# revdotcom/paper_accurate_fast_cheap

Hardware: AMD Instinct MI355X
Metric: audio-sec/sec (1/RTF) GigaSpeech long-form encode (higher is better)
Workload: dtype f32+bf16-slot

## Files before the change

### include/pafc_encoder_ops.h

```cpp
#ifndef PAFC_ENCODER_OPS_H
#define PAFC_ENCODER_OPS_H

#include "pafc_wkv6.h"

#ifdef __cplusplus
extern "C" {
#endif

int pafc_dwconv1d_cl(int dtype, int B, int T_in, int C, int K, int left_pad, int T_out, const void *x,
                     const void *w, const void *bias, void *y, int glu, const int32_t *lens,
                     pafc_stream_t stream);

int pafc_dwconv1d_cl_ex(int dtype, int B, int T_in, int C, int K, int left_pad, int T_out, const void *x, long ldx,
                        const void *w, const void *bias, void *y, int act, const int32_t *lens, pafc_stream_t stream);

int pafc_dwconv1d_cl_ln_silu(int dtype, int B, int T_in, int C, int K, int left_pad, int T_out, const void *x, long ldx,
                             const void *w, const void *bias, const void *gamma, const void *beta, float eps, void *y,
                             const int32_t *lens, pafc_stream_t stream);

size_t pafc_dwconv1d_cl_wgrad_workspace_bytes(int B, int T_out, int C, int K);
int pafc_dwconv1d_cl_wgrad(int dtype, int B, int T_in, int C, int K, int left_pad, int T_out, const void *x, long ldx,
                           const void *dy, float *dw, float *dbias, void *workspace, size_t workspace_bytes,
                           pafc_stream_t stream);

// ... 149 lines not shown
int pafc_mamba2_scan_skip_bf16(int B, int L, int H, const void *xbc, long ldx, const float *dt, const float *log_a,
                               const float *D, void *y_bf16, int reverse, int chunk_len, void *workspace,
                               size_t workspace_bytes, pafc_stream_t stream);
int pafc_mamba2_gate_norm(int dtype, long rows, int d_inner, const void *y, const void *z, long ld_z,
                          const void *norm_weight, float eps, void *out, pafc_stream_t stream);

int pafc_gemm_bf16(long M, int N, int K, int batch, const void *A, long lda, long strideA, const void *W, long ldw,
                   long strideW, const void *bias, long strideBias, const void *residual, long ldr, long strideR,
                   void *out, long ldo, long strideO, float alpha, int act, pafc_stream_t stream);
int pafc_gemm_bf16_glu_half(long M, int N, int K, int batch);
int pafc_conv3x3s2_nhwc_bf16_ph(int B, int T1, int F1, int Ci, int Co, const void *in, const void *w_tap_co_ci, const void *bias,
                                void *out, int relu, int tile_m, pafc_stream_t stream);
int pafc_gemm_bf16_ph(long M, int N, int K, int batch, const void *A, long lda, long strideA, const void *W, long ldw,
                      long strideW, const void *bias, long strideBias, const void *residual, long ldr, long strideR,
                      void *out, long ldo, long strideO, float alpha, int act, int tile_n, int tile_m, pafc_stream_t stream);
int pafc_gemm_ph_ex(long M, int N, int K, int batch, const void *A, long lda, long strideA, int a_split, const void *W, long ldw,
                    long strideW, const void *bias, long strideBias, const void *residual, int res_kind, long ldr, long strideR,
                    void *out, int out_kind, long ldo, long lo_off, long strideO, float alpha, int act, int tile_m,
                    pafc_stream_t stream);
int pafc_gemm_ph_ex2(long M, int N, int K, int batch, const void *A, long lda, long strideA, int a_split, int a_plane_block,
                     const void *W, long ldw, long strideW, const void *bias, long strideBias, const void *residual, int res_kind,
                     long ldr, long strideR, void *out, int out_kind, long ldo, long lo_off, long strideO, float alpha, int act,
                     int tile_m, pafc_stream_t stream);
int pafc_conv3x3s2_nhwc_split_ph(int B, int T1, int F1, int Ci, int Co, const void *in_planes, const void *w3_tap_co_3ci,
                                 const float *bias, void *out_planes, int relu, int tile_m, pafc_stream_t stream);

int pafc_residual_dropout(int backward, int dtype_x, int dtype_y, long n, const void *x, const void *y, void *out, float scale,
                          float p, unsigned long long seed, unsigned long long offset, pafc_stream_t stream);
int pafc_silu_dropout(int backward, int dtype, long n, const void *h, const void *dout, void *out, float p,
                      unsigned long long seed, unsigned long long offset, pafc_stream_t stream);

int pafc_multi_transpose_bf16(const void *table, int n, int total_tiles, pafc_stream_t stream);
int pafc_multi_cast_bf16(const void *table, int n, int total_chunks, pafc_stream_t stream);

#ifdef __cplusplus
}
#endif
#endif
```

### paper_accurate_fast_cheap_amd/csrc/gemm_bf16.hip

```cpp
#include <stdio.h>
#include <stdlib.h>

#include "pafc_common.h"
#include "../../include/pafc_encoder_ops.h"

namespace pafc {
namespace {

constexpr int GBM = 128, GBN = 128, GBK = 64;
typedef float f32x4g __attribute__((ext_vector_type(4)));
typedef __bf16 bf16x8g __attribute__((ext_vector_type(8)));

struct GemmParams {
    const bf16_t *A, *W, *bias, *res;
    bf16_t *out;
    long M;
    int N, K;
    long lda, ldw, ldo, ldr;
    long sA, sW, sO, sB, sR;
    float alpha;
    int act;
    int mtiles, ntiles;
    int nk1, K1;
    int pb_sh;
// ... 285 lines not shown
                        (bf16_t)f32_to_bf16_bits(apply_act(fmaf(acc[i][j][g], p.alpha, bv), p.act));
        }
        __syncthreads();
        constexpr int CPR = BN / 8, RPP = 256 / CPR;
#pragma unroll
        for (int q = 0; q < BM / RPP; ++q) {
            const int row = q * RPP + tid / CPR, c8 = (tid % CPR) * 8;
            const long m = m0 + row;
            if (m < p.M && n0 + c8 < p.N)
                *reinterpret_cast<uint4 *>(Oz + m * p.ldo + n0 + c8) = *reinterpret_cast<const uint4 *>(O + row * LDO + c8);
        }
    }
}

}
}

extern "C" int pafc_gemm_bf16_ph(long M, int N, int K, int batch, const void *A, long lda, long strideA, const void *W, long ldw,
                                 long strideW, const void *bias, long strideBias, const void *residual, long ldr, long strideR,
                                 void *out, long ldo, long strideO, float alpha, int act, int tile_n, int tile_m,
                                 pafc_stream_t stream);

static int ph_tile_m(long M, int N, int K, int batch, int act, bool has_residual) {
    if (N % 8 || K % 128 || N < 256) return 0;
    if (act == 4 && N % 256) return 0;
    if (has_residual && act != 0) return 0;
    const int cus = pafc::device_cus();
    const long nt = (N + 255) / 256;
    static const long min_fill = [] { const char *e = getenv("PAFC_PH_MIN_FILL"); return e ? atol(e) : 0L; }();
    if (min_fill > 0) {
        if (((M + 255) / 256) * nt * batch * 100 < (long)cus * min_fill) return 0;
    } else if (((M + 127) / 128) * ((N + 127) / 128) * batch <= 2L * cus) {
        return 0;
    }
    long best_cost = -1;
    int best = 0;
    for (int tm = 256; tm >= 192; tm -= 64) {
        const long tiles = ((M + tm - 1) / tm) * nt * batch;
        const long cost = ((tiles + cus - 1) / cus) * (tm + 64);
        if (best_cost < 0 || cost < best_cost) { best_cost = cost; best = tm; }
    }
    return best;
}

extern "C" int pafc_gemm_bf16_glu_half(long M, int N, int K, int batch) { return ph_tile_m(M, N, K, batch, 4, false) ? 32 : 64; }

extern "C" int pafc_gemm_bf16(long M, int N, int K, int batch, const void *A, long lda, long strideA, const void *W,
                              long ldw, long strideW, const void *bias, long strideBias, const void *residual, long ldr,
                              long strideR, void *out, long ldo, long strideO, float alpha, int act,
                              pafc_stream_t stream) {
    if (!A || !W || !out) return PAFC_ERR_NULL_POINTER;
    if (M <= 0 || N <= 0 || K <= 0 || batch <= 0 || batch > 65535) return PAFC_ERR_BAD_DIMS;
    if (N % 8 || K % pafc::GBK) return PAFC_ERR_UNSUPPORTED;
    if (act < 0 || act > 4) return PAFC_ERR_UNSUPPORTED;
    if (const int tm = ph_tile_m(M, N, K, batch, act, residual != nullptr)) {
        const int rc = pafc_gemm_bf16_ph(M, N, K, batch, A, lda, strideA, W, ldw, strideW, bias, strideBias, residual, ldr, strideR,
                                         out, ldo, strideO, alpha, act, 256, tm, stream);
        if (rc != PAFC_ERR_UNSUPPORTED) return rc;
        if (act == 4) return PAFC_ERR_UNSUPPORTED;
    }
    const bool glu = act == 4;
    if (glu && (N % pafc::GBN || residual)) return PAFC_ERR_UNSUPPORTED;
    if (lda < K || ldw < K || ldo < (glu ? N / 2 : N) || (residual && ldr < N)) return PAFC_ERR_BAD_DIMS;
    if ((lda | ldw | ldo | strideA | strideW | strideO) % 8 || (residual && ((ldr | strideR) % 8))) return PAFC_ERR_ALIGNMENT;
    if ((((uintptr_t)A | (uintptr_t)W | (uintptr_t)out | (uintptr_t)residual) & 15) != 0) return PAFC_ERR_ALIGNMENT;
    pafc::GemmParams p{};
    p.A = (const pafc::bf16_t *)A; p.W = (const pafc::bf16_t *)W; p.bias = (const pafc::bf16_t *)bias;
    p.res = (const pafc::bf16_t *)residual; p.out = (pafc::bf16_t *)out;
    p.M = M; p.N = N; p.K = K;
    p.lda = lda; p.ldw = ldw; p.ldo = ldo; p.ldr = ldr;
    p.sA = strideA; p.sW = strideW; p.sO = strideO; p.sB = strideBias; p.sR = strideR;
    p.alpha = alpha; p.act = act;
    const long cus = pafc::device_cus();
    auto tiles = [&](int bm, int bn) { return ((M + bm - 1) / bm) * ((N + bn - 1) / bn) * (long)batch; };
    int bm = 128, bn = 128;
    if (!glu && tiles(128, 128) * 5 < 7 * cus) {
        if (tiles(128, 64) >= 2 * cus) bn = 64;
        else { bm = 64; bn = 64; }
// ... 187 lines not shown
```

### paper_accurate_fast_cheap_amd/csrc/gemm_ph.hip

```cpp
#include <climits>
#include <cstdlib>
#include <cstring>
#include <type_traits>

#include "pafc_common.h"
#include "../../include/pafc_encoder_ops.h"

namespace pafc {
namespace {

typedef float f32x4p __attribute__((ext_vector_type(4)));
typedef __bf16 bf16x8p __attribute__((ext_vector_type(8)));
typedef unsigned u32x4p __attribute__((ext_vector_type(4)));

struct PhParams {
    const bf16_t *A, *W;
    const void *bias;
    const void *res;
    void *out;
    long M;
    int N, K;
    long lda, ldw, ldo, ldr;
    long sA, sW, sO, sB, sR;
    float alpha;
    int mtiles, ntiles;
    int tm;
    int batch;
    int nk1, pb_shift;
    long pb_bytes;
    int nsteps, a_lo, w_lo;
    int w_step;
    long lo_off;
    float *ln_stats;
    const float *ln_csum;
    float ln_eps, ln_inv_c;
    int T1, F1, T2, F2, Ci, CiA, CiW, spt, inv_spt;
    long in_bytes;
#ifdef PH_STAMPS
    unsigned long long *stamps;
#endif
};

#ifdef PH_STAMPS
#define PH_STAMP(i) do { if (stamp_on) st[(i)] = __builtin_amdgcn_s_memtime(); } while (0)
#else
#define PH_STAMP(i) do { } while (0)
#endif

__device__ __forceinline__ void dma16(__amdgpu_buffer_rsrc_t rsrc, unsigned lane_off, unsigned uniform_off, void *lds_wave_base) {
    __builtin_amdgcn_raw_ptr_buffer_load_lds(rsrc, (__attribute__((address_space(3))) void *)lds_wave_base, 16, lane_off,
// ... 34 lines not shown
__global__ __launch_bounds__(512, 2) void gemm_ph_kernel(const PhParams p) {
    constexpr int BN = PBN;
    constexpr int UA = 128 * 128;
    constexpr int UB = (BN / 2) * 128;
    constexpr int STEP = 2 * UA + 2 * UB;
    constexpr int OFF_A0 = 0, OFF_A1 = UA, OFF_B0 = 2 * UA, OFF_B1 = 2 * UA + UB;
    constexpr int TN = 2;
    constexpr int DA = UA / 8192;
    constexpr int DB = UB / 8192;
    constexpr int OSZ = OUT == 1 ? 4 : 2;
    constexpr bool BIASF32 = OUT != 0;
    constexpr int NST = 8 * (GLU ? 1 : 2) * (OUT == 0 ? 1 : 2) + (LNF == 2 ? 8 : 0);
    static_assert(LNF == 0 || (OUT == 0 && !CONV), "LayerNorm folding: bf16 GEMMs");
    static_assert(!SPL || LNF == 0, "shared-fragment split operands: not with a folded LayerNorm");
    static_assert(LNF != 1 || (RES == 0 && (GLU || ACT == 1)), "LNF 1: the w_1 (SiLU) / pointwise_conv1 (GLU) projections");
    static_assert(LNF != 2 || RES == 1, "LNF 2: a residual GEMM");
    static_assert(!(GLU && (ACT != 0 || RES != 0)), "GLU excludes an activation and a residual");
    static_assert(!(RES != 0 && ACT != 0), "the layer never pairs a residual with an activation");
    extern __shared__ __attribute__((aligned(1024))) unsigned char lds[];

    const int tid = threadIdx.x, lane = tid & 63;
    const int wave = __builtin_amdgcn_readfirstlane(tid >> 6);
    const int wr = wave >> 2, wc = wave & 3;
    const long nblk = (long)p.mtiles * p.ntiles;
    const long total = nblk * p.batch;
    const long per = total / 8;
    const int nt = SPL ? p.nsteps : p.K / PBK;

    auto pix_off = [&](long m) -> long {
        const long tf = (long)p.T2 * p.F2;
        const long bb = m / tf, rem = m - bb * tf;
        const long t2 = rem / p.F2, f2 = rem - t2 * p.F2;
        return (((bb * p.T1 + 2 * t2) * p.F1 + 2 * f2) * p.CiA) * 2;
    };

    struct Tile {
        long m0;
        int n0, z, vr;
        __amdgpu_buffer_rsrc_t Ar, Wr;
    };
    auto make_tile = [&](long t, Tile &T) {
        const bool real = t < total;
        long tt = real ? t : 0;
        if (tt < per * 8) tt = (tt % 8) * per + tt / 8;
        T.z = (int)(tt / nblk);
        const long bid = tt % nblk;
        const int mt0 = (int)(bid / p.ntiles), nt0 = (int)(bid % p.ntiles);
        T.m0 = (long)mt0 * p.tm;
        T.n0 = nt0 * BN;
        T.vr = (int)min((long)p.tm, p.M - T.m0);
        if constexpr (CONV) {
            const long a_base = pix_off(T.m0);
            T.Ar = make_rsrc(reinterpret_cast<const unsigned char *>(p.A) + a_base, real ? p.in_bytes - a_base : 0);
            T.Wr = make_rsrc(p.W + (long)T.n0 * p.CiW, real ? ((long)8 * p.N + p.N - T.n0) * p.CiW * 2 : 0);
        } else {
            T.Ar = make_rsrc(p.A + T.z * p.sA + T.m0 * p.lda, real ? (p.M - T.m0) * p.lda * 2 : 0);
            T.Wr = make_rsrc(p.W + T.z * p.sW + (long)T.n0 * p.ldw, real ? ((long)(p.N - 1 - T.n0) * p.ldw + p.K) * 2 : 0);
        }
    };

    unsigned a_off[2][DA], b_off[2][DB];
    auto a_offsets = [&](const Tile &T, int h) {
        int sl = lane;
        asm volatile("" : "+v"(sl));
        const int sub = sl >> 3, pch = sl & 7;
#pragma unroll
        for (int j = 0; j < DA; ++j) {
            const int u = (wave * DA + j) * 8 + sub;
            const int row = (u >> 6) * 128 + h * 64 + (u & 63);
            const int sc = pch ^ sub;
            const unsigned coff = SPL ? (unsigned)(16 * (sc & 3) + (sc >> 2) * p.a_lo) : (unsigned)(16 * sc);
            a_off[h][j] = CONV ? (unsigned)(pix_off(T.m0 + row) - pix_off(T.m0)) + coff
                               : (unsigned)((long)row * p.lda * 2) + coff;
        }
    };
    auto b_offsets = [&]() {
        const int sub = lane >> 3, pch = lane & 7;
#pragma unroll
        for (int h = 0; h < 2; ++h)
// ... 446 lines not shown
    first = false;
    if constexpr (CONV) make_tile(t + gridDim.x, cur);
    else cur = nxt;
    PH_STAMP(53);
    }
    PH_WAIT(0);
}

template <bool GLU, int ACT, int RES, int OUT, bool CONV = false, int LNF = 0, bool SPL = false>
int launch_ph(const PhParams &p, int batch, hipStream_t s) {
    constexpr size_t lds = 2 * (2 * 128 * 128 + 2 * (PBN / 2) * 128) + 8 * 1024 + (LNF == 1 ? 8 * 1024 + 16 * 1024 : 0);
    auto kern = gemm_ph_kernel<GLU, ACT, RES, OUT, CONV, LNF, SPL>;
    static bool attr_set[64];
    int dev = 0;
    if (hipGetDevice(&dev) != hipSuccess) return PAFC_ERR_LAUNCH;
    if (dev < 0 || dev >= 64 || !attr_set[dev]) {
        if (hipFuncSetAttribute((const void *)kern, hipFuncAttributeMaxDynamicSharedMemorySize, (int)lds) != hipSuccess)
            return PAFC_ERR_LAUNCH;
        if (dev >= 0 && dev < 64) attr_set[dev] = true;
    }
    const int cus = device_cus();
    PhParams q = p;
    q.batch = batch;
    const long total = (long)p.mtiles * p.ntiles * batch;
    const long grid = total < cus ? total : cus;
    hipLaunchKernelGGL(kern, dim3((unsigned)grid), dim3(512), lds, s, q);
    return hipGetLastError() == hipSuccess ? PAFC_OK : PAFC_ERR_LAUNCH;
}

int g_split_walk = -1;
bool split_shared_fragments() {
    if (g_split_walk < 0) {
        const char *e = getenv("PAFC_SPLIT_WALK");
        g_split_walk = !(e && std::strcmp(e, "hilohi") == 0);
    }
    return g_split_walk != 0;
}

}
}

extern "C" int pafc_gemm_ph_ex(long M, int N, int K, int batch, const void *A, long lda, long strideA, int a_split, const void *W,
                               long ldw, long strideW, const void *bias, long strideBias, const void *residual, int res_kind,
                               long ldr, long strideR, void *out, int out_kind, long ldo, long lo_off, long strideO, float alpha,
                               int act, int tile_m, pafc_stream_t stream) {
    return pafc_gemm_ph_ex2(M, N, K, batch, A, lda, strideA, a_split, 0, W, ldw, strideW, bias, strideBias, residual, res_kind, ldr,
                            strideR, out, out_kind, ldo, lo_off, strideO, alpha, act, tile_m, stream);
}

extern "C" int pafc_gemm_ph_ex2(long M, int N, int K, int batch, const void *A, long lda, long strideA, int a_split,
                                int a_plane_block, const void *W, long ldw, long strideW, const void *bias, long strideBias,
                                const void *residual, int res_kind, long ldr, long strideR, void *out, int out_kind, long ldo,
                                long lo_off, long strideO, float alpha, int act, int tile_m, pafc_stream_t stream) {
    if (!A || !W || !out) return PAFC_ERR_NULL_POINTER;
    if (M <= 0 || N <= 0 || K <= 0 || batch <= 0 || batch > 65535) return PAFC_ERR_BAD_DIMS;
    if (act < 0 || act > 4 || out_kind < 0 || out_kind > 2 || res_kind < 0 || res_kind > 2) return PAFC_ERR_UNSUPPORTED;
    if (!residual) res_kind = 0;
    else if (res_kind == 0) return PAFC_ERR_BAD_DIMS;
    const bool glu = act == 4;
    if (tile_m < 64 || tile_m > 256 || tile_m % 64) return PAFC_ERR_UNSUPPORTED;
    if (N % 8 || K % 128) return PAFC_ERR_UNSUPPORTED;
    if (glu && (N % 256 || residual)) return PAFC_ERR_UNSUPPORTED;
    if (residual && act != 0) return PAFC_ERR_UNSUPPORTED;
    if (res_kind == 1 && out_kind != 0) return PAFC_ERR_UNSUPPORTED;
    if (res_kind == 2 && out_kind != 1) return PAFC_ERR_UNSUPPORTED;
    const int Kw = a_split ? 3 * K : K;
    const int No = glu ? N / 2 : N;
    if (lda < (a_split ? 2 * K : K) || ldw < Kw || (residual && ldr < N)) return PAFC_ERR_BAD_DIMS;
    if (out_kind == 2 ? (lo_off < No || ldo < lo_off + No) : ldo < No) return PAFC_ERR_BAD_DIMS;
    if ((lda | ldw | strideA | strideW) % 8 || (ldo | strideO | lo_off) % 8 || (residual && ((ldr | strideR) % 8))) return PAFC_ERR_ALIGNMENT;
    if ((((uintptr_t)A | (uintptr_t)W | (uintptr_t)out | (uintptr_t)residual | (uintptr_t)bias) & 15) != 0) return PAFC_ERR_ALIGNMENT;
    if ((double)M * lda * 2 >= 2.0e9 || (double)N * ldw * 2 >= 2.0e9) return PAFC_ERR_UNSUPPORTED;
    if ((double)256 * ldo * 4 >= 2.0e9 || (residual && (double)256 * ldr * 4 >= 2.0e9)) return PAFC_ERR_UNSUPPORTED;
    pafc::PhParams p{};
    p.A = (const pafc::bf16_t *)A; p.W = (const pafc::bf16_t *)W; p.bias = bias; p.res = residual; p.out = out;
    p.M = M; p.N = N; p.K = Kw;
    p.lda = lda; p.ldw = ldw; p.ldo = ldo; p.ldr = ldr;
    p.sA = strideA; p.sW = strideW; p.sO = strideO; p.sB = strideBias; p.sR = strideR;
    p.alpha = alpha;
    p.nk1 = a_split ? K / 64 : INT_MAX / 4;
    p.pb_shift = 31;
    p.pb_bytes = (long)K * 2;
    if (a_split && a_plane_block) {
        int sh = 0;
        while ((64 << sh) < a_plane_block) ++sh;
        if ((64 << sh) != a_plane_block || K % a_plane_block) return PAFC_ERR_UNSUPPORTED;
        p.pb_shift = sh;
        p.pb_bytes = (long)a_plane_block * 2;
    }
    p.lo_off = lo_off;
    p.tm = tile_m;
    p.mtiles = (int)((M + tile_m - 1) / tile_m);
    p.ntiles = (N + 255) / 256;
    if ((long)p.mtiles * p.ntiles > 0x7fffffffL) return PAFC_ERR_BAD_DIMS;
    hipStream_t s = (hipStream_t)stream;
    if (a_split && out_kind != 0 && pafc::split_shared_fragments() && (double)2 * K * 2 + 64 < 2.0e9) {
        p.nsteps = K / 32;
        p.a_lo = (int)p.pb_bytes;
        p.w_lo = 2 * K * 2;
        p.w_step = 64;
        p.pb_shift = p.pb_shift >= 30 ? 30 : p.pb_shift + 1;
        if (out_kind == 1) {
            if (glu) return pafc::launch_ph<true, 0, 0, 1, false, 0, true>(p, batch, s);
            if (res_kind == 2) return pafc::launch_ph<false, 0, 2, 1, false, 0, true>(p, batch, s);
            if (act == 0) return pafc::launch_ph<false, 0, 0, 1, false, 0, true>(p, batch, s);
            return PAFC_ERR_UNSUPPORTED;
        }
        if (glu || residual) return PAFC_ERR_UNSUPPORTED;
        if (act == 1) return pafc::launch_ph<false, 1, 0, 2, false, 0, true>(p, batch, s);
        if (act == 0) return pafc::launch_ph<false, 0, 0, 2, false, 0, true>(p, batch, s);
        return PAFC_ERR_UNSUPPORTED;
    }
    if (out_kind == 0) {
        if (glu) return pafc::launch_ph<true, 0, 0, 0>(p, batch, s);
        if (res_kind == 1) return pafc::launch_ph<false, 0, 1, 0>(p, batch, s);
        switch (act) {
            case 1: return pafc::launch_ph<false, 1, 0, 0>(p, batch, s);
            case 2: return pafc::launch_ph<false, 2, 0, 0>(p, batch, s);
            case 3: return pafc::launch_ph<false, 3, 0, 0>(p, batch, s);
            default: return pafc::launch_ph<false, 0, 0, 0>(p, batch, s);
        }
    }
    if (out_kind == 1) {
        if (glu) return pafc::launch_ph<true, 0, 0, 1>(p, batch, s);
        if (res_kind == 2) return pafc::launch_ph<false, 0, 2, 1>(p, batch, s);
        if (act == 0) return pafc::launch_ph<false, 0, 0, 1>(p, batch, s);
        return PAFC_ERR_UNSUPPORTED;
    }
    if (glu || residual) return PAFC_ERR_UNSUPPORTED;
    if (act == 1) return pafc::launch_ph<false, 1, 0, 2>(p, batch, s);
    if (act == 0) return pafc::launch_ph<false, 0, 0, 2>(p, batch, s);
    return PAFC_ERR_UNSUPPORTED;
}

extern "C" int pafc_gemm_bf16_ph_ln(long M, int N, int K, const void *A, long lda, const void *W, long ldw, const void *bias,
                                    const void *residual, long ldr, void *out, long ldo, float alpha, int act, int ln_mode,
                                    float *stats, const float *csum, int ln_c, float ln_eps, int tile_m, pafc_stream_t stream) {
    if (!A || !W || !out || !stats) return PAFC_ERR_NULL_POINTER;
    if (M <= 0 || N <= 0 || K <= 0 || ln_c <= 0) return PAFC_ERR_BAD_DIMS;
    if (tile_m < 64 || tile_m > 256 || tile_m % 64) return PAFC_ERR_UNSUPPORTED;
    if (N % 8 || K % 128) return PAFC_ERR_UNSUPPORTED;
    const bool glu = act == 4;
    if (ln_mode == 1) {
        if (!csum || residual || (act != 1 && act != 4) || alpha != 1.f || K != ln_c) return PAFC_ERR_UNSUPPORTED;
        if (glu && N % 256) return PAFC_ERR_UNSUPPORTED;
    } else if (ln_mode == 2) {
        if (!residual || act != 0 || N != 512 || ln_c != N) return PAFC_ERR_UNSUPPORTED;
    } else {
        return PAFC_ERR_UNSUPPORTED;
    }
    const int No = glu ? N / 2 : N;
    if (lda < K || ldw < K || ldo < No || (residual && ldr < N)) return PAFC_ERR_BAD_DIMS;
    if ((lda | ldw | ldo) % 8 || (residual && ldr % 8)) return PAFC_ERR_ALIGNMENT;
    if ((((uintptr_t)A | (uintptr_t)W | (uintptr_t)out | (uintptr_t)residual | (uintptr_t)bias | (uintptr_t)stats | (uintptr_t)csum) & 15) != 0)
        return PAFC_ERR_ALIGNMENT;
    if ((double)M * lda * 2 >= 2.0e9 || (double)N * ldw * 2 >= 2.0e9 || (double)256 * ldo * 4 >= 2.0e9 ||
        (residual && (double)256 * ldr * 4 >= 2.0e9))
        return PAFC_ERR_UNSUPPORTED;
    pafc::PhParams p{};
    p.A = (const pafc::bf16_t *)A; p.W = (const pafc::bf16_t *)W; p.bias = bias; p.res = residual; p.out = out;
    p.M = M; p.N = N; p.K = K;
    p.lda = lda; p.ldw = ldw; p.ldo = ldo; p.ldr = ldr;
    p.alpha = alpha;
    p.nk1 = INT_MAX / 4; p.pb_shift = 31; p.pb_bytes = (long)K * 2;
    p.ln_stats = stats; p.ln_csum = csum; p.ln_eps = ln_eps; p.ln_inv_c = 1.f / (float)ln_c;
    p.tm = tile_m;
    p.mtiles = (int)((M + tile_m - 1) / tile_m);
    p.ntiles = (N + 255) / 256;
    if ((long)p.mtiles * p.ntiles > 0x7fffffffL) return PAFC_ERR_BAD_DIMS;
    hipStream_t s = (hipStream_t)stream;
    if (ln_mode == 2) return pafc::launch_ph<false, 0, 1, 0, false, 2>(p, 1, s);
    if (glu) return pafc::launch_ph<true, 0, 0, 0, false, 1>(p, 1, s);
    return pafc::launch_ph<false, 1, 0, 0, false, 1>(p, 1, s);
}

extern "C" int pafc_gemm_bf16_ph(long M, int N, int K, int batch, const void *A, long lda, long strideA, const void *W,
                                 long ldw, long strideW, const void *bias, long strideBias, const void *residual, long ldr,
                                 long strideR, void *out, long ldo, long strideO, float alpha, int act, int tile_n,
                                 int tile_m, pafc_stream_t stream) {
    if (tile_n != 256) return PAFC_ERR_UNSUPPORTED;
    return pafc_gemm_ph_ex(M, N, K, batch, A, lda, strideA, 0, W, ldw, strideW, bias, strideBias, residual, residual ? 1 : 0, ldr,
                           strideR, out, 0, ldo, 0, strideO, alpha, act, tile_m, stream);
}

static int conv_ph_launch(int B, int T1, int F1, int Ci, int Co, const void *in, const void *w, const void *bias, void *out,
                          int relu, int tile_m, int split, pafc_stream_t stream) {
    if (!in || !w || !out) return PAFC_ERR_NULL_POINTER;
    if (B <= 0 || T1 < 3 || F1 < 3 || Ci <= 0 || Co <= 0) return PAFC_ERR_BAD_DIMS;
    if (Ci % 128 || Co % 8) return PAFC_ERR_UNSUPPORTED;
    if (tile_m != 256 && tile_m != 192 && tile_m != 128) return PAFC_ERR_UNSUPPORTED;
    if ((((uintptr_t)in | (uintptr_t)w | (uintptr_t)out | (uintptr_t)bias) & 15) != 0) return PAFC_ERR_ALIGNMENT;
    const int T2 = (T1 - 3) / 2 + 1, F2 = (F1 - 3) / 2 + 1;
// ... 43 lines not shown
```

### paper_accurate_fast_cheap_amd/csrc/pafc_common.h

```cpp
#pragma once
#include <hip/hip_runtime.h>
#include <stdint.h>

namespace pafc {

constexpr int kWave = 64;

typedef uint16_t bf16_t;

__device__ __forceinline__ float bf16_bits_to_f32(uint32_t h) { return __uint_as_float(h << 16); }

__device__ __forceinline__ uint32_t f32_to_bf16_bits(float f) {
    return (uint32_t)__builtin_bit_cast(unsigned short, static_cast<__bf16>(f));
}

__device__ __forceinline__ float round_bf16(float f) { return static_cast<float>(static_cast<__bf16>(f)); }

template <typename ET> struct Elem;
template <> struct Elem<float> {
    static constexpr int kPerLane = 4;
    __device__ static __forceinline__ void unpack(const uint4 &q, float *f) {
        f[0] = __uint_as_float(q.x); f[1] = __uint_as_float(q.y);
        f[2] = __uint_as_float(q.z); f[3] = __uint_as_float(q.w);
    }
    __device__ static __forceinline__ float load(const float *p) { return *p; }
// ... 5 lines not shown
    __device__ static __forceinline__ void unpack(const uint4 &q, float *f) {
        f[0] = bf16_bits_to_f32(q.x & 0xffffu); f[1] = __uint_as_float(q.x & 0xffff0000u);
        f[2] = bf16_bits_to_f32(q.y & 0xffffu); f[3] = __uint_as_float(q.y & 0xffff0000u);
        f[4] = bf16_bits_to_f32(q.z & 0xffffu); f[5] = __uint_as_float(q.z & 0xffff0000u);
        f[6] = bf16_bits_to_f32(q.w & 0xffffu); f[7] = __uint_as_float(q.w & 0xffff0000u);
    }
    __device__ static __forceinline__ float load(const bf16_t *p) { return bf16_bits_to_f32(*p); }
    __device__ static __forceinline__ void store(bf16_t *p, float v) { *p = (bf16_t)f32_to_bf16_bits(v); }
    __device__ static __forceinline__ float round(float v) { return round_bf16(v); }
};

inline int device_cus() {
    static int cached[64];
    int dev = 0;
    if (hipGetDevice(&dev) != hipSuccess || dev < 0 || dev >= 64) return 256;
    int c = cached[dev];
    if (c <= 0) {
        if (hipDeviceGetAttribute(&c, hipDeviceAttributeMultiprocessorCount, dev) != hipSuccess || c <= 0) c = 256;
        cached[dev] = c;
    }
    return c;
}

__device__ __forceinline__ float wave_sum(float x) {
#pragma unroll
    for (int off = 32; off > 0; off >>= 1) x += __shfl_xor(x, off, kWave);
    return x;
}

}
```

### paper_accurate_fast_cheap_amd/hip_ops.py

```python
import contextlib
import ctypes
import os
import threading
import weakref
from typing import Optional

import torch

from . import _lib
from ._lib import c_int, c_void_p


DISPATCH = dict(skinny_max_rows=640, own_gemm_min_rows=1, lds_resident_min_rows=8192, split_gemm_min_rows=1024,
                ln_fold_min_rows=24576, dwconv_ln_silu_max_rows=24575, split_small_max_rows=8192, split_layers_min_rows=256)


def _load_dispatch():
    legacy = dict(skinny_max_rows="PAFC_SKINNY_MAX_ROWS", own_gemm_min_rows="PAFC_OWN_GEMM_MIN_ROWS",
                  lds_resident_min_rows="PAFC_LDS_RESIDENT_MIN_ROWS", split_gemm_min_rows="PAFC_SPLIT_GEMM_MIN_ROWS")
    for name, env in legacy.items():
        if os.environ.get(env):
            DISPATCH[name] = int(os.environ[env])
    for item in filter(None, os.environ.get("PAFC_DISPATCH", "").split(",")):
        name, _, value = item.partition("=")
# ... 1110 lines not shown
    _lib.require_gpu(bias, stats, csum)
    for t in (a, w, residual, out):
        if t is not None and (not t.is_cuda or t.dtype != torch.bfloat16 or t.stride(-1) != 1 or t.dim() != 2):
            raise _lib.PafcError("gemm_bf16_ln: 2-d bf16 GPU tensors with unit stride in the last dimension")
    M, K = a.shape
    N = w.shape[0]
    No = N // 2 if act == "glu" else N
    if stats.dtype != torch.float32 or stats.numel() != M * 16 or not stats.is_contiguous():
        raise _lib.PafcError("gemm_bf16_ln: stats is a contiguous float32 (M, 8, 2) buffer")
    if out is None:
        out = torch.empty((M, No), dtype=a.dtype, device=a.device)
    L = _bind2()
    if not getattr(L, "_pafc_gemmln_bound", False):
        from ctypes import c_float, c_long
        P, I, G = c_void_p, c_int, c_long
        _lib._sig(L.pafc_gemm_bf16_ph_ln, I, G, I, I, P, G, P, G, P, P, G, P, G, c_float, I, I, P, P, I, c_float, I, P)
        L._pafc_gemmln_bound = True
    from .profiling import op_timer
    with op_timer("gemm_%dx%d" % (K, N), sample=12, flops=2.0 * M * N * K):
        rc = L.pafc_gemm_bf16_ph_ln(M, N, K, _lib.ptr(a), a.stride(0), _lib.ptr(w), w.stride(0), _lib.ptr(bias), _lib.ptr(residual),
                                    residual.stride(0) if residual is not None else 0, _lib.ptr(out), out.stride(0), float(alpha),
                                    _ACTS[act], 1 if csum is not None else 2, _lib.ptr(stats), _lib.ptr(csum),
                                    int(ln_c or (K if csum is not None else N)),
                                    float(eps), _ph_tile_m(M, N, min_tm=128), _lib.stream_of(a))
    _lib.check(rc, "pafc_gemm_bf16_ph_ln")
    return out


def split_planes(x: torch.Tensor, triple: bool = False) -> torch.Tensor:
    _lib.require_gpu(x)
    if x.dtype != torch.float32 or x.stride(-1) != 1:
        raise _lib.PafcError("split_planes: contiguous fp32 input")
    K = x.shape[-1]
    rows = x.numel() // K
    out = torch.empty(x.shape[:-1] + ((3 if triple else 2) * K,), dtype=torch.bfloat16, device=x.device)
    L = _bind2()
    if not getattr(L, "_pafc_split_planes_bound", False):
        from ctypes import c_long
        _lib._sig(L.pafc_split_planes, c_int, c_long, c_int, c_void_p, c_long, c_void_p, c_long, c_long, c_int, c_void_p)
        L._pafc_split_planes_bound = True
    _lib.check(L.pafc_split_planes(rows, K, _lib.ptr(x), K, _lib.ptr(out), out.shape[-1], K, int(triple), _lib.stream_of(x)),
               "pafc_split_planes")
    return out


def _ph_tile_m(M: int, N: int, batch: int = 1, min_tm: int = 64) -> int:
    cus = torch.cuda.get_device_properties(torch.cuda.current_device()).multi_processor_count
    nt = (N + 255) // 256
    best = None
    for tm in (256, 192, 128, 64):
        if tm < min_tm:
            continue
        tiles = ((M + tm - 1) // tm) * nt * batch
        cost = ((tiles + cus - 1) // cus) * (tm + 64)
        if best is None or cost < best[0]:
            best = (cost, tm)
    return best[1]


def gemm_ph_ex(a: torch.Tensor, w: torch.Tensor, bias: Optional[torch.Tensor] = None, act: str = "none", alpha: float = 1.0,
               residual: Optional[torch.Tensor] = None, out: Optional[torch.Tensor] = None, a_split: bool = False,
               out_kind: str = "bf16", tile_m: int = 0, a_plane_block: int = 0) -> torch.Tensor:
    _lib.require_gpu(bias)
    for t in (a, w, residual, out):
        if t is not None and (not t.is_cuda or t.stride(-1) != 1):
            raise _lib.PafcError("gemm_ph_ex: GPU tensors with unit stride in the last dimension")
    if a.dtype != torch.bfloat16 or w.dtype != torch.bfloat16 or a.dim() != 2 or w.dim() != 2:
        raise _lib.PafcError("gemm_ph_ex: a and w are 2-d bf16 (planes of fp32 operands with a_split)")
    M = a.shape[0]
    N = w.shape[0]
    K = w.shape[1] // 3 if a_split else w.shape[1]
    if a.shape[1] != (2 * K if a_split else K) or (a_split and w.shape[1] != 3 * K):
        raise _lib.PafcError("gemm_ph_ex: a (M, K) x w (N, K); split: a (M, 2K) x w (N, 3K)")
    No = N // 2 if act == "glu" else N
    kinds = {"bf16": (0, torch.bfloat16, No), "f32": (1, torch.float32, No), "planes": (2, torch.bfloat16, 2 * No)}
    ok, odt, ocols = kinds[out_kind]
    if out is None:
        out = torch.empty((M, ocols), dtype=odt, device=a.device)
    if out.dtype != odt or tuple(out.shape) != (M, ocols):
        raise _lib.PafcError("gemm_ph_ex: out must be (M, N) in the output form's dtype ((M, 2N) bf16 for planes)")
# ... 10 lines not shown
        P, I, G = c_void_p, c_int, c_long
        _lib._sig(L.pafc_gemm_ph_ex2, I, G, I, I, I, P, G, G, I, I, P, G, G, P, G, P, I, G, G, P, I, G, G, G, c_float, I, I, P)
        from ctypes import c_size_t
        _lib._sig(L.pafc_gemm_bf16_f32out_pb, I, G, I, I, P, G, I, I, P, G, P, P, G, P, I, G, G, c_float, I, P, c_size_t, P)
        _lib._sig(L.pafc_gemm_bf16_f32out_workspace_bytes, c_size_t, G, I, I, I)
        L._pafc_gemmex_bound = True
    from .profiling import op_timer
    pb_ok = not a_plane_block or (a_split and a_plane_block >= 64 and a_plane_block & (a_plane_block - 1) == 0 and K % a_plane_block == 0)
    if (M <= _SPLIT_SMALL_MAX_ROWS and M * N <= _SPLIT_SMALL_MAX_OUT and ok != 0 and act in ("none", "silu", "tanh", "relu")
            and pb_ok and not tile_m and K % 64 == 0):
        nws = L.pafc_gemm_bf16_f32out_workspace_bytes(M, N, K, int(a_split))
        ws = torch.empty(nws, dtype=torch.uint8, device=a.device) if nws else None
        with op_timer("gemm%ss_%dx%d" % ("3" if a_split else "", K, N), sample=12, flops=2.0 * M * N * K * (3 if a_split else 1)):
            rc = L.pafc_gemm_bf16_f32out_pb(M, N, K, _lib.ptr(a), a.stride(0), int(a_split), int(a_plane_block), _lib.ptr(w), w.stride(0),
                                            _lib.ptr(bias), _lib.ptr(residual), residual.stride(0) if residual is not None else 0,
                                            _lib.ptr(out), ok, out.stride(0), No if ok == 2 else 0, float(alpha), _ACTS[act], _lib.ptr(ws),
                                            nws, _lib.stream_of(a))
        _lib.check(rc, "pafc_gemm_bf16_f32out")
        return out
    with op_timer("gemm%s_%dx%d" % ("3" if a_split else "", K, N), sample=12, flops=2.0 * M * N * K * (3 if a_split else 1)):
        rc = L.pafc_gemm_ph_ex2(M, N, K, 1, _lib.ptr(a), a.stride(0), 0, int(a_split), int(a_plane_block), _lib.ptr(w), w.stride(0), 0,
                                _lib.ptr(bias), 0,
                               _lib.ptr(residual), rk, residual.stride(0) if residual is not None else 0, 0, _lib.ptr(out), ok,
                               out.stride(0), No if ok == 2 else 0, 0, float(alpha), _ACTS[act], int(tile_m or _ph_tile_m(M, N)),
                               _lib.stream_of(a))
    _lib.check(rc, "pafc_gemm_ph_ex")
    return out


_SPLIT_SMALL_MAX_ROWS = DISPATCH["split_small_max_rows"]
_SPLIT_SMALL_MAX_OUT = 1 << 22


def wkv6_single_chunk(B: int, T: int, C: int, H: int) -> bool:
    return _lib.lib().pafc_wkv6_pick_chunk_len(B, T, C, H, 1) >= T


def _check_prev(prev: Optional[torch.Tensor], x: torch.Tensor):
    if prev is not None and (prev.dtype != x.dtype or prev.numel() != x.shape[0] * x.shape[2] or not prev.is_contiguous()
                             or prev.device != x.device):
        raise _lib.PafcError("tmix: prev must be a contiguous (B, C) tensor of x's dtype on x's device")


def tmix_shift_mix(x: torch.Tensor, maa_x0: torch.Tensor, maa_x1: Optional[torch.Tensor], reverse0: bool = False,
                   prev: Optional[torch.Tensor] = None):
    _lib.require_gpu(x, maa_x0, maa_x1, prev)
    _check_prev(prev, x)
# ... 866 lines not shown
    _lib.require_gpu(x, w1, b1, w2_3, b2)
    B, T, Fd = x.shape
    C = w1.shape[0]
    if x.dtype != torch.float32 or w1.dtype != torch.float32 or w2_3.dtype != torch.bfloat16 or tuple(w2_3.shape) != (9, C, 3 * C):
        raise _lib.PafcError("conv_sub_f32split_planes: fp32 x (B, T, F) / w1, w2 as (9, C, 3C) bf16 planes")
    L = _bind()
    if not getattr(L, "_pafc_splitph_bound", False):
        from ctypes import c_long
        P, I = c_void_p, c_int
        _lib._sig(L.pafc_conv3x3s2_c1_nhwc_f32split_ps, I, I, I, I, I, P, P, P, P, P, c_long, I, P)
        _lib._sig(L.pafc_conv3x3s2_nhwc_split_ph, I, I, I, I, I, I, P, P, P, P, I, I, P)
        L._pafc_splitph_bound = True
    T1, F1 = (T - 3) // 2 + 1, (Fd - 3) // 2 + 1
    T2, F2 = (T1 - 3) // 2 + 1, (F1 - 3) // 2 + 1
    y1 = torch.empty((B, T1, F1, 2 * C), dtype=torch.bfloat16, device=x.device)
    st = _lib.stream_of(x)
    lo = c_void_p(y1.data_ptr() + 2 * C)
    _lib.check(L.pafc_conv3x3s2_c1_nhwc_f32split_ps(B, T, Fd, C, _lib.ptr(x), _lib.ptr(w1), _lib.ptr(b1), _lib.ptr(y1), lo, 2 * C, 1, st),
               "pafc_conv3x3s2_c1_nhwc_f32split_ps")
    out = torch.empty((B, T2, F2, 2 * C), dtype=torch.bfloat16, device=x.device)
    from .profiling import op_timer
    with op_timer("conv3x3s2_split", flops=2.0 * B * T2 * F2 * C * 9 * C * 3):
        rc = L.pafc_conv3x3s2_nhwc_split_ph(B, T1, F1, C, C, _lib.ptr(y1), _lib.ptr(w2_3), _lib.ptr(b2), _lib.ptr(out), 1,
                                            _ph_tile_m(B * T2 * F2, C, min_tm=128), st)
    _lib.check(rc, "pafc_conv3x3s2_nhwc_split_ph")
    return out


def _bind_mamba():
    L = _bind()
    if not getattr(L, "_pafc_mamba_bound", False):
        from ctypes import c_float, c_long
        P, I, G = c_void_p, c_int, c_long
        _lib._sig(L.pafc_dwconv1d_cl_ex, I, I, I, I, I, I, I, I, P, G, P, P, P, I, P, P)
        _lib._sig(L.pafc_mamba2_prep, I, I, I, I, I, P, P, G, P, P, P, P, P, P, P, P, P)
        _lib._sig(L.pafc_mamba2_finish, I, I, I, I, I, P, P, P, P, G, P, G, P, P, P, c_float, I, P, P)
        from ctypes import c_size_t
        _lib._sig(L.pafc_mamba2_scan_workspace_bytes, c_size_t, I, I, I, I)
        _lib._sig(L.pafc_mamba2_scan, I, I, I, I, P, G, P, P, P, I, P, c_size_t, P)
        _lib._sig(L.pafc_mamba2_scan_dir, I, I, I, I, P, G, P, P, P, I, I, P, c_size_t, P)
        _lib._sig(L.pafc_mamba2_scan_skip_bf16, I, I, I, I, P, G, P, P, P, P, I, I, P, c_size_t, P)
        _lib._sig(L.pafc_mamba2_gate_norm, I, I, G, I, P, P, G, P, c_float, P, P)
        L._pafc_mamba_bound = True
    return L


def causal_conv_silu_cl(x: torch.Tensor, weight: torch.Tensor, bias: Optional[torch.Tensor], reverse: bool = False
# ... 77 lines not shown
```

Before: 47850.

## Plan persistent GEMM tiles with cost model and mixed two-height M tiling

Measured after the change: 48380, median of 6. 1.01x the previous value.

```diff
diff --git a/include/pafc_encoder_ops.h b/include/pafc_encoder_ops.h
--- a/include/pafc_encoder_ops.h
+++ b/include/pafc_encoder_ops.h
@@ -195,6 +195,10 @@
                      const void *W, long ldw, long strideW, const void *bias, long strideBias, const void *residual, int res_kind,
                      long ldr, long strideR, void *out, int out_kind, long ldo, long lo_off, long strideO, float alpha, int act,
                      int tile_m, pafc_stream_t stream);
+#define PAFC_PH_PLAN_SPLIT 1
+#define PAFC_PH_PLAN_ONE_HEIGHT 2
+#define PAFC_PH_PLAN_UNCLIPPED 4
+int pafc_gemm_ph_plan(long M, int N, int K, int batch, int cus, int min_tm, int flags, int *plan);
 int pafc_conv3x3s2_nhwc_split_ph(int B, int T1, int F1, int Ci, int Co, const void *in_planes, const void *w3_tap_co_3ci,
                                  const float *bias, void *out_planes, int relu, int tile_m, pafc_stream_t stream);
 
diff --git a/paper_accurate_fast_cheap_amd/csrc/gemm_bf16.hip b/paper_accurate_fast_cheap_amd/csrc/gemm_bf16.hip
--- a/paper_accurate_fast_cheap_amd/csrc/gemm_bf16.hip
+++ b/paper_accurate_fast_cheap_amd/csrc/gemm_bf16.hip
@@ -331,28 +331,23 @@
                                  pafc_stream_t stream);
 
 static int ph_tile_m(long M, int N, int K, int batch, int act, bool has_residual) {
-    if (N % 8 || K % 128 || N < 256) return 0;
-    if (act == 4 && N % 256) return 0;
-    if (has_residual && act != 0) return 0;
+    if (N % 8 || K % 128 || N < 256) return -1;
+    if (act == 4 && N % 256) return -1;
+    if (has_residual && act != 0) return -1;
     const int cus = pafc::device_cus();
     const long nt = (N + 255) / 256;
     static const long min_fill = [] { const char *e = getenv("PAFC_PH_MIN_FILL"); return e ? atol(e) : 0L; }();
     if (min_fill > 0) {
-        if (((M + 255) / 256) * nt * batch * 100 < (long)cus * min_fill) return 0;
+        if (((M + 255) / 256) * nt * batch * 100 < (long)cus * min_fill) return -1;
     } else if (((M + 127) / 128) * ((N + 127) / 128) * batch <= 2L * cus) {
-        return 0;
-    }
-    long best_cost = -1;
-    int best = 0;
-    for (int tm = 256; tm >= 192; tm -= 64) {
-        const long tiles = ((M + tm - 1) / tm) * nt * batch;
-        const long cost = ((tiles + cus - 1) / cus) * (tm + 64);
-        if (best_cost < 0 || cost < best_cost) { best_cost = cost; best = tm; }
-    }
-    return best;
-}
-
-extern "C" int pafc_gemm_bf16_glu_half(long M, int N, int K, int batch) { return ph_tile_m(M, N, K, batch, 4, false) ? 32 : 64; }
+        return -1;
+    }
+    int plan[4];
+    pafc_gemm_ph_plan(M, N, K, batch, cus, 192, PAFC_PH_PLAN_UNCLIPPED, plan);
+    return plan[0];
+}
+
+extern "C" int pafc_gemm_bf16_glu_half(long M, int N, int K, int batch) { return ph_tile_m(M, N, K, batch, 4, false) >= 0 ? 32 : 64; }
 
 extern "C" int pafc_gemm_bf16(long M, int N, int K, int batch, const void *A, long lda, long strideA, const void *W,
                               long ldw, long strideW, const void *bias, long strideBias, const void *residual, long ldr,
@@ -362,7 +357,7 @@
     if (M <= 0 || N <= 0 || K <= 0 || batch <= 0 || batch > 65535) return PAFC_ERR_BAD_DIMS;
     if (N % 8 || K % pafc::GBK) return PAFC_ERR_UNSUPPORTED;
     if (act < 0 || act > 4) return PAFC_ERR_UNSUPPORTED;
-    if (const int tm = ph_tile_m(M, N, K, batch, act, residual != nullptr)) {
+    if (const int tm = ph_tile_m(M, N, K, batch, act, residual != nullptr); tm >= 0) {
         const int rc = pafc_gemm_bf16_ph(M, N, K, batch, A, lda, strideA, W, ldw, strideW, bias, strideBias, residual, ldr, strideR,
                                          out, ldo, strideO, alpha, act, 256, tm, stream);
         if (rc != PAFC_ERR_UNSUPPORTED) return rc;
diff --git a/paper_accurate_fast_cheap_amd/csrc/gemm_ph.hip b/paper_accurate_fast_cheap_amd/csrc/gemm_ph.hip
--- a/paper_accurate_fast_cheap_amd/csrc/gemm_ph.hip
+++ b/paper_accurate_fast_cheap_amd/csrc/gemm_ph.hip
@@ -26,6 +26,8 @@
     int mtiles, ntiles;
     int tm;
     int batch;
+    int a_to_end;
+    int mt1, tm2, mt2;
     int nk1, pb_shift;
     long pb_bytes;
     int nsteps, a_lo, w_lo;
@@ -106,9 +108,9 @@
     const int tid = threadIdx.x, lane = tid & 63;
     const int wave = __builtin_amdgcn_readfirstlane(tid >> 6);
     const int wr = wave >> 2, wc = wave & 3;
-    const long nblk = (long)p.mtiles * p.ntiles;
-    const long total = nblk * p.batch;
-    const long per = total / 8;
+    const int nblk1 = p.mt1 * p.ntiles, nblk2 = p.mt2 * p.ntiles;
+    const int total1 = nblk1 * p.batch;
+    const long total = total1 + nblk2 * p.batch;
     const int nt = SPL ? p.nsteps : p.K / PBK;
 
     auto pix_off = [&](long m) -> long {
@@ -125,20 +127,26 @@
     };
     auto make_tile = [&](long t, Tile &T) {
         const bool real = t < total;
-        long tt = real ? t : 0;
-        if (tt < per * 8) tt = (tt % 8) * per + tt / 8;
-        T.z = (int)(tt / nblk);
-        const long bid = tt % nblk;
-        const int mt0 = (int)(bid / p.ntiles), nt0 = (int)(bid % p.ntiles);
-        T.m0 = (long)mt0 * p.tm;
+        int tt = real ? (int)t : 0;
+        const bool seg2 = tt >= total1;
+        const int nblk = seg2 ? nblk2 : nblk1;
+        if (seg2) tt -= total1;
+        const int per = (nblk * p.batch) >> 3;
+        if (tt < per * 8) tt = (tt & 7) * per + (tt >> 3);
+        T.z = tt / nblk;
+        const int bid = tt - T.z * nblk;
+        const int mt0 = bid / p.ntiles, nt0 = bid - mt0 * p.ntiles;
+        const int h = seg2 ? p.tm2 : p.tm;
+        T.m0 = seg2 ? (long)p.mt1 * p.tm + (long)mt0 * h : (long)mt0 * h;
         T.n0 = nt0 * BN;
-        T.vr = (int)min((long)p.tm, p.M - T.m0);
+        T.vr = (int)min((long)h, p.M - T.m0);
         if constexpr (CONV) {
             const long a_base = pix_off(T.m0);
             T.Ar = make_rsrc(reinterpret_cast<const unsigned char *>(p.A) + a_base, real ? p.in_bytes - a_base : 0);
             T.Wr = make_rsrc(p.W + (long)T.n0 * p.CiW, real ? ((long)8 * p.N + p.N - T.n0) * p.CiW * 2 : 0);
         } else {
-            T.Ar = make_rsrc(p.A + T.z * p.sA + T.m0 * p.lda, real ? (p.M - T.m0) * p.lda * 2 : 0);
+            const long a_rows = p.a_to_end ? p.M - T.m0 : T.vr;
+            T.Ar = make_rsrc(p.A + T.z * p.sA + T.m0 * p.lda, real ? a_rows * p.lda * 2 : 0);
             T.Wr = make_rsrc(p.W + T.z * p.sW + (long)T.n0 * p.ldw, real ? ((long)(p.N - 1 - T.n0) * p.ldw + p.K) * 2 : 0);
         }
     };
@@ -631,6 +639,7 @@
     const int cus = device_cus();
     PhParams q = p;
     q.batch = batch;
+    if (q.mt1 == 0 && q.mt2 == 0) q.mt1 = q.mtiles;
     const long total = (long)p.mtiles * p.ntiles * batch;
     const long grid = total < cus ? total : cus;
     hipLaunchKernelGGL(kern, dim3((unsigned)grid), dim3(512), lds, s, q);
@@ -646,7 +655,89 @@
     return g_split_walk != 0;
 }
 
-}
+constexpr int PLAN_H[4] = {256, 192, 128, 64};
+constexpr int PLAN_KS_SPLIT[4] = {3490, 3100, 2720, 2280};
+constexpr int PLAN_KS_BF16[4] = {2880, 2690, 2560, 2360};
+constexpr int PLAN_FIX[4] = {20000, 18000, 15000, 12000};
+
+long plan_makespan(long tiles1, long c1, long tiles2, long c2, int cus) {
+    const long total = tiles1 + tiles2, grid = total < cus ? total : cus;
+    auto n = [&](long T, long b) { return T > b ? (T - 1 - b) / grid + 1 : 0L; };
+    long worst = 0;
+    for (long b : {0L, tiles1 % grid, total % grid}) {
+        if (b >= grid) continue;
+        const long n1 = n(tiles1, b), load = n1 * c1 + (n(total, b) - n1) * c2;
+        if (load > worst) worst = load;
+    }
+    return worst;
+}
+
+}
+
+int ph_plan(long M, int N, int K, int batch, int cus, int min_tm, int flags, int plan[4]) {
+    const long nt = (N + 255) / 256;
+    if (cus <= 0) cus = 1;
+    long best = -1;
+    plan[0] = 256; plan[1] = (int)((M + 255) / 256); plan[2] = 0; plan[3] = 0;
+    if (flags & PAFC_PH_PLAN_UNCLIPPED) {
+        for (int i = 0; i < 4 && PLAN_H[i] >= min_tm; ++i) {
+            const int tm = PLAN_H[i];
+            const long tiles = ((M + tm - 1) / tm) * nt * batch;
+            const long cost = ((tiles + cus - 1) / cus) * (tm + 64);
+            if (best < 0 || cost < best) { best = cost; plan[0] = tm; plan[1] = (int)((M + tm - 1) / tm); }
+        }
+        return PAFC_OK;
+    }
+    const bool split = flags & PAFC_PH_PLAN_SPLIT;
+    const long nsteps = split ? K / 32 : K / 64;
+    long cost[4];
+    for (int i = 0; i < 4; ++i) cost[i] = nsteps * (split ? PLAN_KS_SPLIT[i] : PLAN_KS_BF16[i]) + PLAN_FIX[i];
+    for (int i = 0; i < 4 && PLAN_H[i] >= min_tm; ++i) {
+        const int tm = PLAN_H[i];
+        const long mt = (M + tm - 1) / tm;
+        const long c = plan_makespan(mt * nt * batch, cost[i], 0, 0, cus);
+        if (best < 0 || c < best) { best = c; plan[0] = tm; plan[1] = (int)mt; plan[2] = 0; plan[3] = 0; }
+        if (flags & PAFC_PH_PLAN_ONE_HEIGHT) continue;
+        for (int j = i + 1; j < 4 && PLAN_H[j] >= min_tm; ++j) {
+            const int tm2 = PLAN_H[j];
+            for (long mt1 = M / tm; mt1 >= 1; --mt1) {
+                const long rest = M - mt1 * tm, mt2 = (rest + tm2 - 1) / tm2;
+                if (mt2 * nt * batch > 2L * cus) break;
+                if (mt2 == 0) continue;
+                const long c2 = plan_makespan(mt1 * nt * batch, cost[i], mt2 * nt * batch, cost[j], cus);
+                if (c2 < best) { best = c2; plan[0] = tm; plan[1] = (int)mt1; plan[2] = tm2; plan[3] = (int)mt2; }
+            }
+        }
+    }
+    return PAFC_OK;
+}
+
+bool ph_set_tiles(PhParams &p, long M, int N, int K, int batch, int tile_m, int min_tm, bool split) {
+    const bool legacy = ph_plan_legacy();
+    int plan[4] = {tile_m, (int)((M + (tile_m ? tile_m : 1) - 1) / (tile_m ? tile_m : 1)), 0, 0};
+    if (tile_m == 0)
+        ph_plan(M, N, K, batch, device_cus(), min_tm,
+                legacy || !split ? PAFC_PH_PLAN_UNCLIPPED | PAFC_PH_PLAN_ONE_HEIGHT : PAFC_PH_PLAN_SPLIT, plan);
+    p.a_to_end = legacy;
+    p.tm = plan[0]; p.mt1 = plan[1]; p.tm2 = plan[2]; p.mt2 = plan[3];
+    p.mtiles = p.mt1 + p.mt2;
+    p.ntiles = (N + 255) / 256;
+    if (p.tm < 64 || p.tm > 256 || p.tm % 64 || p.mt1 < 1) return false;
+    if (p.mt2 ? (p.tm2 < 64 || p.tm2 >= p.tm || p.tm2 % 64 || (long)p.mt1 * p.tm >= M || (long)p.mt1 * p.tm + (long)p.mt2 * p.tm2 < M ||
+                 (long)p.mt1 * p.tm + (long)(p.mt2 - 1) * p.tm2 >= M)
+              : (long)p.mt1 * p.tm < M || (long)(p.mt1 - 1) * p.tm >= M)
+        return false;
+    return (long)p.mtiles * p.ntiles * batch <= 0x7fffffffL;
+}
+
+}
+
+extern "C" int pafc_gemm_ph_plan(long M, int N, int K, int batch, int cus, int min_tm, int flags, int *plan) {
+    if (!plan) return PAFC_ERR_NULL_POINTER;
+    if (M <= 0 || N <= 0 || K <= 0 || batch <= 0) return PAFC_ERR_BAD_DIMS;
+    if (min_tm != 64 && min_tm != 128 && min_tm != 192 && min_tm != 256) return PAFC_ERR_UNSUPPORTED;
+    if (flags & ~7) return PAFC_ERR_UNSUPPORTED;
+    return pafc::ph_plan(M, N, K, batch, cus > 0 ? cus : pafc::device_cus(), min_tm, flags, plan);
 }
 
 extern "C" int pafc_gemm_ph_ex(long M, int N, int K, int batch, const void *A, long lda, long strideA, int a_split, const void *W,
@@ -667,7 +758,7 @@
     if (!residual) res_kind = 0;
     else if (res_kind == 0) return PAFC_ERR_BAD_DIMS;
     const bool glu = act == 4;
-    if (tile_m < 64 || tile_m > 256 || tile_m % 64) return PAFC_ERR_UNSUPPORTED;
+    if (tile_m != 0 && (tile_m < 64 || tile_m > 256 || tile_m % 64)) return PAFC_ERR_UNSUPPORTED;
     if (N % 8 || K % 128) return PAFC_ERR_UNSUPPORTED;
     if (glu && (N % 256 || residual)) return PAFC_ERR_UNSUPPORTED;
     if (residual && act != 0) return PAFC_ERR_UNSUPPORTED;
@@ -698,12 +789,10 @@
         p.pb_bytes = (long)a_plane_block * 2;
     }
     p.lo_off = lo_off;
-    p.tm = tile_m;
-    p.mtiles = (int)((M + tile_m - 1) / tile_m);
-    p.ntiles = (N + 255) / 256;
-    if ((long)p.mtiles * p.ntiles > 0x7fffffffL) return PAFC_ERR_BAD_DIMS;
+    const bool spl = a_split && out_kind != 0 && pafc::split_shared_fragments() && (double)2 * K * 2 + 64 < 2.0e9;
+    if (!pafc::ph_set_tiles(p, M, N, a_split && !spl ? 3 * K : K, batch, tile_m, 64, spl)) return PAFC_ERR_BAD_DIMS;
     hipStream_t s = (hipStream_t)stream;
-    if (a_split && out_kind != 0 && pafc::split_shared_fragments() && (double)2 * K * 2 + 64 < 2.0e9) {
+    if (spl) {
         p.nsteps = K / 32;
         p.a_lo = (int)p.pb_bytes;
         p.w_lo = 2 * K * 2;
@@ -747,7 +836,7 @@
                                     float *stats, const float *csum, int ln_c, float ln_eps, int tile_m, pafc_stream_t stream) {
     if (!A || !W || !out || !stats) return PAFC_ERR_NULL_POINTER;
     if (M <= 0 || N <= 0 || K <= 0 || ln_c <= 0) return PAFC_ERR_BAD_DIMS;
-    if (tile_m < 64 || tile_m > 256 || tile_m % 64) return PAFC_ERR_UNSUPPORTED;
+    if (tile_m != 0 && (tile_m < 64 || tile_m > 256 || tile_m % 64)) return PAFC_ERR_UNSUPPORTED;
     if (N % 8 || K % 128) return PAFC_ERR_UNSUPPORTED;
     const bool glu = act == 4;
     if (ln_mode == 1) {
@@ -773,10 +862,7 @@
     p.alpha = alpha;
     p.nk1 = INT_MAX / 4; p.pb_shift = 31; p.pb_bytes = (long)K * 2;
     p.ln_stats = stats; p.ln_csum = csum; p.ln_eps = ln_eps; p.ln_inv_c = 1.f / (float)ln_c;
-    p.tm = tile_m;
-    p.mtiles = (int)((M + tile_m - 1) / tile_m);
-    p.ntiles = (N + 255) / 256;
-    if ((long)p.mtiles * p.ntiles > 0x7fffffffL) return PAFC_ERR_BAD_DIMS;
+    if (!pafc::ph_set_tiles(p, M, N, K, 1, tile_m, 128, false)) return PAFC_ERR_BAD_DIMS;
     hipStream_t s = (hipStream_t)stream;
     if (ln_mode == 2) return pafc::launch_ph<false, 0, 1, 0, false, 2>(p, 1, s);
     if (glu) return pafc::launch_ph<true, 0, 0, 0, false, 1>(p, 1, s);
diff --git a/paper_accurate_fast_cheap_amd/csrc/pafc_common.h b/paper_accurate_fast_cheap_amd/csrc/pafc_common.h
--- a/paper_accurate_fast_cheap_amd/csrc/pafc_common.h
+++ b/paper_accurate_fast_cheap_amd/csrc/pafc_common.h
@@ -1,6 +1,8 @@
 #pragma once
 #include <hip/hip_runtime.h>
 #include <stdint.h>
+#include <cstdlib>
+#include <cstring>
 
 namespace pafc {
 
@@ -52,6 +54,11 @@
     return c;
 }
 
+inline bool ph_plan_legacy() {
+    static const bool legacy = [] { const char *e = getenv("PAFC_PH_PLAN"); return e && e[0] == 'l' && !strcmp(e, "legacy"); }();
+    return legacy;
+}
+
 __device__ __forceinline__ float wave_sum(float x) {
 #pragma unroll
     for (int off = 32; off > 0; off >>= 1) x += __shfl_xor(x, off, kWave);
diff --git a/paper_accurate_fast_cheap_amd/hip_ops.py b/paper_accurate_fast_cheap_amd/hip_ops.py
--- a/paper_accurate_fast_cheap_amd/hip_ops.py
+++ b/paper_accurate_fast_cheap_amd/hip_ops.py
@@ -1156,7 +1156,7 @@
                                     residual.stride(0) if residual is not None else 0, _lib.ptr(out), out.stride(0), float(alpha),
                                     _ACTS[act], 1 if csum is not None else 2, _lib.ptr(stats), _lib.ptr(csum),
                                     int(ln_c or (K if csum is not None else N)),
-                                    float(eps), _ph_tile_m(M, N, min_tm=128), _lib.stream_of(a))
+                                    float(eps), 0, _lib.stream_of(a))
     _lib.check(rc, "pafc_gemm_bf16_ph_ln")
     return out
 
@@ -1178,18 +1178,15 @@
     return out
 
 
-def _ph_tile_m(M: int, N: int, batch: int = 1, min_tm: int = 64) -> int:
-    cus = torch.cuda.get_device_properties(torch.cuda.current_device()).multi_processor_count
-    nt = (N + 255) // 256
-    best = None
-    for tm in (256, 192, 128, 64):
-        if tm < min_tm:
-            continue
-        tiles = ((M + tm - 1) // tm) * nt * batch
-        cost = ((tiles + cus - 1) // cus) * (tm + 64)
-        if best is None or cost < best[0]:
-            best = (cost, tm)
-    return best[1]
+def _ph_tile_m(M: int, N: int, K: int, batch: int = 1, min_tm: int = 64, flags: int = 0) -> int:
+    L = _bind2()
+    if not getattr(L, "_pafc_phplan_bound", False):
+        from ctypes import POINTER, c_long
+        _lib._sig(L.pafc_gemm_ph_plan, c_int, c_long, c_int, c_int, c_int, c_int, c_int, c_int, POINTER(c_int))
+        L._pafc_phplan_bound = True
+    plan = (c_int * 4)()
+    _lib.check(L.pafc_gemm_ph_plan(M, N, K, batch, 0, min_tm, flags, plan), "pafc_gemm_ph_plan")
+    return plan[0]
 
 
 def gemm_ph_ex(a: torch.Tensor, w: torch.Tensor, bias: Optional[torch.Tensor] = None, act: str = "none", alpha: float = 1.0,
@@ -1246,7 +1243,7 @@
         rc = L.pafc_gemm_ph_ex2(M, N, K, 1, _lib.ptr(a), a.stride(0), 0, int(a_split), int(a_plane_block), _lib.ptr(w), w.stride(0), 0,
                                 _lib.ptr(bias), 0,
                                _lib.ptr(residual), rk, residual.stride(0) if residual is not None else 0, 0, _lib.ptr(out), ok,
-                               out.stride(0), No if ok == 2 else 0, 0, float(alpha), _ACTS[act], int(tile_m or _ph_tile_m(M, N)),
+                               out.stride(0), No if ok == 2 else 0, 0, float(alpha), _ACTS[act], int(tile_m),
                                _lib.stream_of(a))
     _lib.check(rc, "pafc_gemm_ph_ex")
     return out
@@ -2159,7 +2156,7 @@
     from .profiling import op_timer
     with op_timer("conv3x3s2_split", flops=2.0 * B * T2 * F2 * C * 9 * C * 3):
         rc = L.pafc_conv3x3s2_nhwc_split_ph(B, T1, F1, C, C, _lib.ptr(y1), _lib.ptr(w2_3), _lib.ptr(b2), _lib.ptr(out), 1,
-                                            _ph_tile_m(B * T2 * F2, C, min_tm=128), st)
+                                            _ph_tile_m(B * T2 * F2, C, 9 * C, min_tm=128, flags=6), st)
     _lib.check(rc, "pafc_conv3x3s2_nhwc_split_ph")
     return out
 
```
